# lijun9250lj/video-steganography-PCAMV

Hardware: AMD Instinct MI355X
Metric: 1080p macroblocks/s (embed on) (higher is better)
Workload: dtype u8

## Files before the change

### video-steganography-pcamv_amd/csrc/pcamv_common.h

```cpp
#ifndef PCAMV_COMMON_H
#define PCAMV_COMMON_H
#include <stddef.h>
#include <stdint.h>
#include "../../include/pcamv_gpu.h"
#include "pcamv_variant.h"

#ifdef PCAMV_HOST_EMU
#define PCAMV_DEV static inline
#define PCAMV_CONST static const
#else
#include <hip/hip_runtime.h>
#define PCAMV_DEV __device__ __forceinline__
#define PCAMV_CONST __device__ static const
#endif

#define PCAMV_PAD 32
#define PCAMV_CPAD 16
#define PCAMV_LSW 28
#define PCAMV_LROW 32
#define PCAMV_LSTRIPS(stride) (((stride) + PCAMV_LSW - 1) / PCAMV_LSW + 1)
#define PCAMV_LSTRIP_OF(x) (((uint32_t)(x) * 18725u) >> 19)
#define PCAMV_COST_MAX (1 << 28)
#define PCAMV_COST_MV_LEN (4 * 4 * 2048 + 1)
#define PCAMV_COST_MV_CENTRE (2 * 4 * 2048)
// ... 101 lines not shown
    int nnz_mask;
    uint32_t cxy[64];
    int ccost[192];
    int slots[16];
    uint8_t recb[24 * 16];
    uint8_t recb0[24 * 16];
    uint8_t pred[24 * 16];
    union {
        struct {
            int16_t coef[24][16];
            int16_t cdc[2][4];
            int blk_nz[24], blk_score[24];
            int red[64];
        };
        uint8_t pred4[4][24 * 16];
    };
    int mvc16[9][2];
    int nbc[12];
    uint32_t win[(4 * 480 + 2 * 192) / 4];
    int win_x0, win_y0, win_cx0, win_cy0;
    uint8_t ib_top[3][28];
    uint8_t ib_left[3][16];
    uint8_t nzc[48];
    int16_t cmvd[48][2];
    int8_t i4mode[48];
    int cbp_left, cbp_top;
    int b_fast_intra, fenc_satd_sum, fenc_sa8d_sum;
    uint8_t snap_pred[24 * 16];
    uint8_t snap_nzc[48];
    int16_t snap_cmvd[48][2];
    int snap_cbp_luma, snap_cbp_chroma, snap_nnz_mask;
    int snap_part, snap_cost;
    uint32_t snap_mv[16];
    int snap_ssd, snap_f8r;
#if defined(PCAMV_PROF)
    uint32_t prof_mv[4][16];
    int prof_ntrial;
#endif
#ifdef PCAMV_SEARCH_CALL
    const struct FrameDev *fdesc;
    int me_tmp[10];
    int mvc_tmp[9][2];
#endif
};
#define PCAMV_PASS2_LDS ((int)offsetof(MBLocal, coef))
#define PCAMV_WAVE_LDS_MAX 10240
static_assert(offsetof(MBLocal, pred) + sizeof(((MBLocal *)0)->pred) == offsetof(MBLocal, coef), "pred must end at the second pass' LDS cut");
static_assert(offsetof(MBLocal, fenc) < PCAMV_PASS2_LDS && offsetof(MBLocal, cmv) < PCAMV_PASS2_LDS && offsetof(MBLocal, cref) < PCAMV_PASS2_LDS &&
              offsetof(MBLocal, nnz_mask) < PCAMV_PASS2_LDS && offsetof(MBLocal, slots) + sizeof(((MBLocal *)0)->slots) <= PCAMV_PASS2_LDS &&
              offsetof(MBLocal, ccost) + sizeof(((MBLocal *)0)->ccost) <= PCAMV_PASS2_LDS, "a field the second pass uses lies beyond its LDS");
static_assert(offsetof(MBLocal, ccost) == offsetof(MBLocal, cxy) + sizeof(((MBLocal *)0)->cxy), "cxy and ccost must be contiguous (cab_residual_walk)");
static_assert(offsetof(MBLocal, recb0) == offsetof(MBLocal, recb) + 384 && offsetof(MBLocal, pred) == offsetof(MBLocal, recb) + 768 &&
              offsetof(MBLocal, coef) == offsetof(MBLocal, recb) + 1152, "recb, recb0, pred, the union must be contiguous in this order (TESA_SLOT, L_IFD)");
#define PCAMV_CHAIN_NZ 464
#define PCAMV_CHAIN_MVD 488
#define PCAMV_CHAIN_BYTES 576
#define L_CAB(L, k) ((uint8_t *)(L)->win + 464 * (k))
#define PCAMV_CAB_USED 276
#define L_CABT(L) ((uint8_t *)(L)->win + 464)
#define L_CABK(L) ((uint8_t *)(L)->win + 464 + PCAMV_CAB_USED)
#define L_CTAB(L) ((L)->win + 256)
#define L_IFD(L) ((uint8_t *)(L)->recb)
#define IFD(L, x, y) (L_IFD(L)[((y) + 1) * 32 + (x) + 4])
PCAMV_DEV int scan8_all_of(int idx)
{
    if (idx < 16) return scan8_of(idx);
    if (idx < 24) return 1 + ((idx - 16) & 1) + 8 * (1 + (((idx - 16) >> 1) & 1) + 3 * ((idx - 16) >> 2));
    return 4 + (idx - 24) + 5 * 8;
}

#define TESA_MAX_RANGE 16
#define TESA_REGION_A ((int)((3 * 24 * 16 + 4 * 24 * 16) / 4))
#define TESA_SLOT(L, i) ((i) < TESA_REGION_A ? (uint32_t *)((uint8_t *)(L) + offsetof(MBLocal, recb)) + (i) : (L)->win + ((i) - TESA_REGION_A))
#define TESA_PACK(sad, ry, rx) ((uint32_t)(sad) << 12 | (uint32_t)(ry) << 6 | (uint32_t)(rx))
#define TESA_SAD(e) ((int)((e) >> 12))
#define NB_LEFT 1
#define NB_TOP 2
#define NB_TOPRIGHT 4
#define NB_TOPLEFT 8

#define CAND_PACK(X, Y) ((uint32_t)(uint16_t)(X) | ((uint32_t)(uint16_t)(Y) << 16))
#define CAND_NONE 0x80008000u
#define CAND_X(c) ((int)(int16_t)(L->cxy[c] & 0xffffu))
#define CAND_Y(c) ((int)(int16_t)(L->cxy[c] >> 16))
#define EV_SATD 1
#define EV_CHROMA 2
#define EV_FPEL 4
#define EV_NOMV 8
#define EV_PROBE 16
#define EV_WIN 32
#define EV_SRC4 64
#define WIN_LW 24
#define WIN_LH 20
#define WIN_LP (WIN_LW * WIN_LH)
#define WIN_CW 16
#define WIN_CH 12
#define WIN_CP (WIN_CW * WIN_CH)
struct EvalRes { int cost, idx; };
#ifdef PCAMV_HOST_EMU
#define FOR_CAND(c, n) for (int c = 0; c < (n); c++)
#define NB_SLOT(i) (i)
#else
#define FOR_CAND(c, n) for (int c = LANE(), c##_1 = 1; c##_1 && c < (n); c##_1 = 0)
#define NB_SLOT(i) 0
#endif

#ifdef PCAMV_HOST_EMU
#define NB_ST32(p, v) (*(uint32_t *)(p) = (uint32_t)(v))
#define NB_ST16(p, v) (*(uint16_t *)(p) = (uint16_t)(v))
#define NB_ST8(p, v) (*(int8_t *)(p) = (int8_t)(v))
#define NB_LD32(p) (*(const uint32_t *)(p))
#define NB_LD8(p) (*(const int8_t *)(p))
#define NB_LD16(p) (*(const uint16_t *)(p))
#else
#define NB_ST32(p, v) __hip_atomic_store((uint32_t *)(p), (uint32_t)(v), __ATOMIC_RELAXED, __HIP_MEMORY_SCOPE_AGENT)
#define NB_ST16(p, v) __hip_atomic_store((uint16_t *)(p), (uint16_t)(v), __ATOMIC_RELAXED, __HIP_MEMORY_SCOPE_AGENT)
#define NB_ST8(p, v) __hip_atomic_store((int8_t *)(p), (int8_t)(v), __ATOMIC_RELAXED, __HIP_MEMORY_SCOPE_AGENT)
#define NB_LD32(p) __hip_atomic_load((uint32_t *)(p), __ATOMIC_RELAXED, __HIP_MEMORY_SCOPE_AGENT)
#define NB_LD8(p) __hip_atomic_load((int8_t *)(p), __ATOMIC_RELAXED, __HIP_MEMORY_SCOPE_AGENT)
#define NB_LD16(p) __hip_atomic_load((uint16_t *)(p), __ATOMIC_RELAXED, __HIP_MEMORY_SCOPE_AGENT)
#endif
#define NB_PACK16(lo, hi) ((uint32_t)(uint16_t)(lo) | (uint32_t)(uint16_t)(hi) << 16)

#ifdef PCAMV_HOST_EMU
#define PCAMV_WAVE_SYNC() do { } while (0)
#else
#define PCAMV_WAVE_SYNC() do { __builtin_amdgcn_fence(__ATOMIC_RELEASE, "wavefront"); __builtin_amdgcn_wave_barrier(); \
                               __builtin_amdgcn_fence(__ATOMIC_ACQUIRE, "wavefront"); } while (0)
#endif

struct MEState {
    int i_pixel, xoff, yoff;
    int mvp[2];
    int cost_mv, cost, cost_rec;
    int mv[2];
};


#if defined(PCAMV_PROF) && !defined(PCAMV_HOST_EMU)
#define PCAMV_PROF_N 48
static __device__ unsigned long long pcamv_prof[PCAMV_PROF_N];
__shared__ unsigned long long pcamv_prof_l[PCAMV_PROF_N];
#define PROF_T() __builtin_readcyclecounter()
#define PROF_ADD(i, t0) do { if ((threadIdx.x & 63) == 0) pcamv_prof_l[i] += (unsigned long long)(PROF_T() - (t0)); } while (0)
// ... 12 lines not shown
```

### video-steganography-pcamv_amd/csrc/pcamv_logic.h

```cpp
#ifndef PCAMV_LOGIC_H
#define PCAMV_LOGIC_H
#include "pcamv_common.h"

PCAMV_DEV void cache_mv_set(MBLocal *L, int x, int y, int w, int h, int mvx, int mvy)
{
    PCAMV_WAVE_SYNC();
    FOR_CAND(i, w * h) {
        int j = i / w, k = i - j * w, idx = SCAN8_0 + x + k + 8 * (y + j);
        L->cmv[idx][0] = (int16_t)mvx; L->cmv[idx][1] = (int16_t)mvy;
    }
    PCAMV_WAVE_SYNC();
}
PCAMV_DEV void cache_ref_set(MBLocal *L, int x, int y, int w, int h, int ref)
{
    PCAMV_WAVE_SYNC();
    FOR_CAND(i, w * h) { int j = i / w, k = i - j * w; L->cref[SCAN8_0 + x + k + 8 * (y + j)] = (int8_t)ref; }
    PCAMV_WAVE_SYNC();
}

PCAMV_DEV void predict_from3(int ref, int refa, int refb, int refc, const int16_t *a, const int16_t *b, const int16_t *c, int mvp[2])
{
    int cnt = (refa == ref) + (refb == ref) + (refc == ref);
    if (cnt > 1) { mvp[0] = median3i(a[0], b[0], c[0]); mvp[1] = median3i(a[1], b[1], c[1]); }
    else if (cnt == 1) {
// ... 901 lines not shown
        mvc[2][0] = a->mvc[i + 3][0]; mvc[2][1] = a->mvc[i + 3][1];
        cache_ref_set(L, 2 * i, 0, 2, 4, 0);
        predict_mv(L, 4 * i, 2, me.mvp);
        me_search<VARIANT>(F, L, &me, mvc, 3);
        a->me8x16[i] = me;
        cache_mv_set(L, 2 * i, 0, 2, 4, me.mv[0], me.mv[1]);
    }
    a->cost8x16 = a->me8x16[0].cost + a->me8x16[1].cost;
}
template <int VARIANT>
PCAMV_DEV void analyse_sub8x8(const FrameDev &F, MBLocal *L, Analysis *a, int i8, int pixel)
{
    L->i_partition = PCAMV_D_8x8;
    int n = pixel == PIX_4x4 ? 4 : 2, cost = 0;
    for (int k = 0; k < n; k++) {
        int idx = 4 * i8 + (pixel == PIX_8x4 ? 2 * k : k);
        MEState *me = pixel == PIX_4x4 ? &a->me4x4[i8][k] : pixel == PIX_8x4 ? &a->me8x4[i8][k] : &a->me4x8[i8][k];
        me_setup(me, pixel, 4 * blk_x_of(idx), 4 * blk_y_of(idx));
        predict_mv(L, idx, pixel == PIX_8x4 ? 2 : 1, me->mvp);
        int mvc[1][2];
        const MEState *cand = pixel == PIX_4x4 ? &a->me8x8[i8] : &a->me4x4[i8][0];
        mvc[0][0] = cand->mv[0]; mvc[0][1] = cand->mv[1];
        me_search<VARIANT>(F, L, me, mvc, k == 0);
        cache_mv_set(L, blk_x_of(idx), blk_y_of(idx), pixel == PIX_8x4 ? 2 : 1, pixel == PIX_4x8 ? 2 : 1, me->mv[0], me->mv[1]);
        cost += me->cost;
    }
    cost += F.lambda * (pixel == PIX_4x4 ? 5 : 3);
    if (F.b_chroma_me) {
        int qx[4], qy[4];
        for (int q = 0; q < 4; q++) {
            const MEState *m4 = pixel == PIX_4x4 ? &a->me4x4[i8][q] : pixel == PIX_8x4 ? &a->me8x4[i8][q >> 1] : &a->me4x8[i8][q & 1];
            qx[q] = m4->mv[0]; qy[q] = m4->mv[1];
        }
        cost += prim_chroma4x4_cost(F, L, i8, qx, qy, F.subme > 1);
    }
    if (pixel == PIX_4x4) a->cost4x4[i8] = cost; else if (pixel == PIX_8x4) a->cost8x4[i8] = cost; else a->cost4x8[i8] = cost;
}

PCAMV_DEV int d_mv_x(int i) { return nib64(0x013443101232ull, i) - 2; }
PCAMV_DEV int d_mv_y(int i) { return nib64(0x100134432321ull, i) - 2; }
PCAMV_DEV int d_nb_x(int i) { return nib64(0x122000121ull, i) - 1; }
PCAMV_DEV int d_nb_y(int i) { return nib64(0x120201210ull, i) - 1; }

PCAMV_DEV int rca_nine(const FrameDev &F, MBLocal *L, MEState *me, const uint8_t *enc, int cx, int cy, int nb_cost, int *last, int win)
{
    const int flags = (F.subme > 1 ? EV_SATD : 0) | ((F.b_chroma_me && me->i_pixel <= PIX_8x8) ? EV_CHROMA : 0) | (win ? EV_WIN : 0);
    FOR_CAND(c, 9) L->cxy[c] = CAND_PACK(cx + d_nb_x(c), cy + d_nb_y(c));
    EvalRes r = eval_cands(F, L, me, enc, 9, flags);
    if (nb_cost) { FOR_CAND(c, 9) L->nbc[c] = L->ccost[c]; PCAMV_WAVE_SYNC(); }
    *last = L->ccost[8];
    return r.cost;
}

PCAMV_DEV int rca_mv_cost(const FrameDev &F, MBLocal *L, Analysis *a, MEState *me, int *m_x, int *m_y, int have_base, int win = 0)
{
    const float beta1 = 1.4, beta2 = 4;
    int bmx = me->mv[0], bmy = me->mv[1];
    int cost = 0, min_cost;
    int b_1_neighbor = 0, b_error_pos = 0;
    if (!have_base) { update_cache(L, a); mb_encode(F, L); prim_copy_pred(L, L->recb0); }
    const unsigned long long t_n = PROF_T();
    min_cost = rca_nine(F, L, me, L->recb0, bmx, bmy, 1, &cost, win);
    PROF_ADD(35, t_n);
    me->cost_rec = L->nbc[8];
    const int want_optimal = !(min_cost < me->cost_rec);
    min_cost = PCAMV_COST_MAX; *m_x = 0; *m_y = 0;
    int ii_best = -1;
    if (win) {
        const int flags = (F.subme > 1 ? EV_SATD : 0) | (F.b_chroma_me ? EV_CHROMA : 0) | EV_WIN | EV_SRC4;
        for (int grp = 0; grp < 3; grp++) {
            PROF_CNT(40, 1);
            const unsigned long long t_g = PROF_T();
            for (int j = 0; j < 4; j++) prim_predict_win16(F, L, j, bmx + d_mv_x(4 * grp + j), bmy + d_mv_y(4 * grp + j));
            prim_mb_transform4(F, L);
            PROF_ADD(36, t_g);
            const unsigned long long t_l = PROF_T();
            FOR_CAND(c, 36) {
                int k = c >> 2, ii = 4 * grp + (c & 3);
                L->cxy[c] = CAND_PACK(bmx + d_mv_x(ii) + d_nb_x(k), bmy + d_mv_y(ii) + d_nb_y(k));
            }
            eval_cands(F, L, me, L->pred4[0], 36, flags);
            PROF_ADD(37, t_l);
            for (int j = 0; j < 4; j++) {
                const int ii = 4 * grp + j;
                int min1 = PCAMV_COST_MAX;
                for (int k = 0; k < 9; k++) min1 = imin(min1, L->ccost[4 * k + j]);
                cost = L->ccost[4 * 8 + j];
                int is_opt = (min1 == cost);
                if (is_opt == want_optimal && cost < min_cost) { min_cost = cost; *m_x = d_mv_x(ii); *m_y = d_mv_y(ii); ii_best = ii; }
            }
            if (grp == 0 && min_cost != PCAMV_COST_MAX) break;
        }
    } else
    for (int ii = 0; ii < 12; ii++) {
        PROF_CNT(41, 1);
        int bx1 = bmx + d_mv_x(ii), by1 = bmy + d_mv_y(ii);
        me->mv[0] = bx1; me->mv[1] = by1;
        update_cache(L, a); mb_encode(F, L, win); prim_copy_pred(L, L->recb);
        int min1 = rca_nine(F, L, me, L->recb, bx1, by1, 0, &cost, win);
        int is_opt = (min1 == cost);
        if (is_opt == want_optimal && cost < min_cost) { min_cost = cost; *m_x = d_mv_x(ii); *m_y = d_mv_y(ii); ii_best = ii; }
        if (ii == 3 && min_cost != PCAMV_COST_MAX) break;
    }
    if (min_cost == PCAMV_COST_MAX) {
        b_error_pos = 1; b_1_neighbor = 1;
        *m_x = 0; *m_y = 0;
        for (int k = 0; k < 4; k++) if (L->nbc[k] < min_cost) { min_cost = L->nbc[k]; *m_x = d_nb_x(k); *m_y = d_nb_y(k); }
    } else b_1_neighbor = ii_best <= 3;
    int cost_opt = min_cost > me->cost_rec ? min_cost - me->cost_rec : 1;
    if (!b_1_neighbor) cost_opt = (int)(beta1 * (float)cost_opt);
    else if (b_error_pos) cost_opt = (int)(beta2 * (float)cost_opt);
    me->mv[0] = bmx; me->mv[1] = bmy;
    update_cache(L, a);
    return cost_opt;
}

PCAMV_DEV int carrier_slots(int i_type, int i_partition, const uint8_t *sub, int used, int slots[16])
{
    int n = 0;
    if (!used) return 0;
    if (i_type == PCAMV_P_8x8) {
        for (int i = 0; i < 4; i++)
            switch (sub[i]) {
            case PCAMV_D_L0_8x8: slots[n++] = i * 4; break;
            case PCAMV_D_L0_4x8: slots[n++] = i * 4; slots[n++] = i * 4 + 1; break;
            case PCAMV_D_L0_8x4: slots[n++] = i * 4; slots[n++] = i * 4 + 2; break;
            default: for (int j = 0; j < 4; j++) slots[n++] = i * 4 + j; break;
            }
    } else if (i_type == PCAMV_P_L0) {
        if (i_partition == PCAMV_D_16x16) slots[n++] = 0;
        else if (i_partition == PCAMV_D_8x16) { slots[n++] = 0; slots[n++] = 4; }
        else if (i_partition == PCAMV_D_16x8) { slots[n++] = 0; slots[n++] = 8; }
    }
    return n;
}

PCAMV_DEV int carrier_of_block(int i_type, int i_partition, const uint8_t *sub, int i)
{
    if (i_type == PCAMV_P_8x8) {
        const int i8 = i >> 2, j = i & 3;
        switch (sub[i8]) {
        case PCAMV_D_L0_8x8: return 4 * i8;
        case PCAMV_D_L0_4x8: return 4 * i8 + (j & 1);
        case PCAMV_D_L0_8x4: return 4 * i8 + (j & 2);
        default: return i;
        }
    }
    if (i_partition == PCAMV_D_8x16) return blk_x_of(i) < 2 ? 0 : 4;
    if (i_partition == PCAMV_D_16x8) return blk_y_of(i) < 2 ? 0 : 8;
    return 0;
}

template <int VARIANT>
PCAMV_DEV int analyse_s16(const FrameDev &F, MBLocal *L, Analysis *a)
{
    int b_skip = 0, b_try_pskip = 0;
    for (int i = 0; i < 4; i++) L->sub_part[i] = PCAMV_D_L0_8x8;
    L->i_partition = PCAMV_D_16x16;
    a->rd16x16 = a->cost8x8 = a->cost16x8 = a->cost8x16 = PCAMV_COST_MAX;
    for (int i = 0; i < 4; i++) a->cost4x4[i] = a->cost8x4[i] = a->cost4x8[i] = PCAMV_COST_MAX;
    a->rd16_early = 0;
    L->snap_part = -1; L->snap_cost = PCAMV_COST_MAX;
#if defined(PCAMV_PROF) && !defined(PCAMV_HOST_EMU)
    L->prof_ntrial = 0;
// ... 140 lines not shown
```

### video-steganography-pcamv_amd/csrc/pcamv_mbkernels.h

```cpp
#ifndef PCAMV_MBKERNELS_H
#define PCAMV_MBKERNELS_H
#include "pcamv_logic.h"

#ifdef PCAMV_HOST_EMU
#define PCAMV_LANE0 1
#define PCAMV_RFL(x) (x)
#else
#define PCAMV_LANE0 (LANE() == 0)
#define PCAMV_RFL(x) rfl(x)
#endif

template <int VARIANT>
PCAMV_DEV void mbk_search_finish(const FrameDev &F, MBLocal *L, Analysis *a, int mb_x, int mb_y)
{
    if (MBRD_ON) {
        const unsigned long long t_c = PROF_T();
        L->b_skip_mc = 0;
        const int kept = L->i_type != PCAMV_P_SKIP && L->snap_part == L->i_partition;
        if (kept) prim_rd_restore(F, L);
        else mb_encode(F, L, 0, 1);
#ifdef PCAMV_HOST_EMU
        prim_store_rec(F, L);
#else
        prim_store_rec(F, L, true);
// ... 65 lines not shown
    for (int k = 0; k < n; k++) {
        int s = slots[k], ip, xo, yo;
        MEState *me = slot_me(L, a, s);
        slot_geometry(L->i_type, L->i_partition, L->sub_part, s, &ip, &xo, &yo);
        me_setup(me, ip, xo, yo);
        me->mv[0] = r->mv[s][0]; me->mv[1] = r->mv[s][1];
        me->mvp[0] = FD(F).mvp_aux[(xy * 16 + s) * 2]; me->mvp[1] = FD(F).mvp_aux[(xy * 16 + s) * 2 + 1];
    }
    return n;
}

PCAMV_DEV void mbk_rca(const FrameDev &F, MBLocal *L, Analysis *a, int xy, int k)
{
    if (!FD(F).rec_mb[xy].used) return;
    int *slots = L->slots;
    const int n = analysis_from_record(F, L, a, xy, slots);
    if (k >= n) return;
    MEState *me = slot_me(L, a, slots[k]);
    int dx = 0, dy = 0;
    const int bx = me->mv[0], by = me->mv[1];
    const int cost = rca_mv_cost(F, L, a, me, &dx, &dy, 0);
    if (PCAMV_LANE0) {
        pcamv_mb_t *r = &FD(F).rec_mb[xy];
        r->mv_stego[slots[k]][0] = (int16_t)(bx + dx); r->mv_stego[slots[k]][1] = (int16_t)(by + dy);
        r->inter_stego_cost[slots[k]] = cost;
    }
}

PCAMV_DEV int mbk_recon(const FrameDev &F, MBLocal *L, Analysis *a, int xy, int fused = 0, int have_rec = 0)
{
    const unsigned long long t_e = PROF_T();
    int n;
    if (fused) {
        L->b_skip_mc = 0;
        n = carrier_slots(L->i_type, L->i_partition, L->sub_part, L->i_type != PCAMV_P_SKIP, L->slots);
        for (int k = 0; k < n; k++) { MEState *me = slot_me(L, a, L->slots[k]); me->cost = me->cost_mv = me->cost_rec = 0; }
        if (have_rec) { PROF_ADD(10, t_e); return n; }
    } else {
        n = analysis_from_record(F, L, a, xy, L->slots);
        update_cache(L, a);
    }
    mb_encode(F, L);
    prim_store_rec(F, L);
    if (PCAMV_LANE0 && FD(F).nnz) FD(F).nnz[xy] = (uint16_t)L->nnz_mask;
    PROF_ADD(10, t_e);
    return n;
}
PCAMV_DEV void mbk_rca_all(const FrameDev &F, MBLocal *L, Analysis *a, int xy, int n)
{
    int *slots = L->slots;
    if (FD(F).rec_mb[xy].used && n > 0) {
        const unsigned long long t_w = PROF_T();
        PROF_CNT(42, n);
        prim_copy_pred(L, L->recb0);
        int win = 0;
        if (L->i_type == PCAMV_P_L0 && L->i_partition == PCAMV_D_16x16) {
            const int bx = a->me16x16.mv[0], by = a->me16x16.mv[1];
            if (bx - 3 >= L->mv_min[0] && bx + 3 <= L->mv_max[0] && by - 3 >= L->mv_min[1] && by + 3 <= L->mv_max[1]) { prim_win_load(F, L, bx, by); win = 1; }
        }
        PROF_ADD(34, t_w);
        for (int k = 0; k < n; k++) {
            MEState *me = slot_me(L, a, slots[k]);
            int dx = 0, dy = 0;
            const int bx = me->mv[0], by = me->mv[1];
            const int cost = rca_mv_cost(F, L, a, me, &dx, &dy, 1, win);
            if (PCAMV_LANE0) {
                pcamv_mb_t *r = &FD(F).rec_mb[xy];
                r->mv_stego[slots[k]][0] = (int16_t)(bx + dx); r->mv_stego[slots[k]][1] = (int16_t)(by + dy);
                r->inter_stego_cost[slots[k]] = cost;
            }
        }
    }
}
PCAMV_DEV void mbk_rca_encode(const FrameDev &F, MBLocal *L, Analysis *a, int xy, int fused = 0, int have_rec = 0)
{
    mbk_rca_all(F, L, a, xy, mbk_recon(F, L, a, xy, fused, have_rec));
}

struct P2Pre { const pcamv_mb_t *r; int base, any_flip, nnz1, drain; };
PCAMV_DEV int mbk_pass2(const FrameDev &F, MBLocal *L, int mb_x, int mb_y, int store_rec = 1, const P2Pre *unit = nullptr)
{
    const int xy = mb_y * F.mb_w + mb_x;
    const pcamv_mb_t *r = unit ? unit->r : (const pcamv_mb_t *)L->ccost;
    PCAMV_WAVE_SYNC();
#ifndef PCAMV_HOST_EMU
    uint32_t pre_y = 0, pre_c = 0;
    int any_flip = 1;
    if (unit) any_flip = unit->any_flip;
    else {
        const int lane = LANE();
        if (FD(F).rec_is_pass1) {
            pre_y = *(const uint32_t *)(FD(F).rec[0] + (size_t)(mb_y * 16 + (lane >> 2)) * FD(F).w + mb_x * 16 + (lane & 3) * 4);
            if (lane < 32) pre_c = *(const uint32_t *)(((lane >> 4) ? FD(F).rec[2] : FD(F).rec[1]) + (size_t)(mb_y * 8 + ((lane & 15) >> 1)) * (FD(F).w >> 1) + mb_x * 8 + (lane & 1) * 4);
        }
        if (FD(F).mbflip) any_flip = FD(F).mbflip[xy];
    }
#else
    const int any_flip = 1;
#endif
    if (!unit) {
        FOR_CAND(i, (int)(sizeof(pcamv_mb_t) / 4) + 1) {
            if (i < (int)(sizeof(pcamv_mb_t) / 4)) ((uint32_t *)L->ccost)[i] = ((const uint32_t *)&FD(F).rec_mb[xy])[i];
            else L->ccost[191] = FD(F).car_base ? FD(F).car_base[xy] : 0;
        }
    }
    PCAMV_WAVE_SYNC();
#ifndef PCAMV_HOST_EMU
    if (unit && unit->drain && r->i_type == PCAMV_P_SKIP) asm volatile("s_waitcnt vmcnt(0)" ::: "memory");
#endif
    const int defer_fenc = unit != nullptr && r->i_type != PCAMV_P_SKIP;
    mb_load(F, L, mb_x, mb_y, r->i_type != PCAMV_P_SKIP ? (defer_fenc ? 2 : 1) : 0);
    L->i_type = r->i_type; L->i_partition = r->i_partition;
// ... 73 lines not shown
```

### video-steganography-pcamv_amd/csrc/pcamv_prims_gpu.h

```cpp
#ifndef PCAMV_PRIMS_GPU_H
#define PCAMV_PRIMS_GPU_H
#include "pcamv_common.h"

__device__ __forceinline__ int pcamv_lane_id(void) { int l = (int)(threadIdx.x & 63); asm volatile("" : "+v"(l)); return l; }
#ifndef PCAMV_RD_LO
#define PCAMV_RD_LO 0
#endif
#define LANE() (PCAMV_RD_LO ? (int)(threadIdx.x & 63) : pcamv_lane_id())
__device__ __forceinline__ uint32_t clamp_u8(int v)
{
    asm volatile("" : "+v"(v));
    return (uint32_t)(v < 0 ? 0 : v > 255 ? 255 : v);
}
__device__ __forceinline__ uint32_t ld4u(const uint8_t *p) { uint32_t v; __builtin_memcpy(&v, p, 4); return v; }
__device__ __forceinline__ uint32_t lds4(const uint8_t *p) { return *(const uint32_t *)p; }
__device__ __forceinline__ void sts4(uint8_t *p, uint32_t v) { *(uint32_t *)p = v; }
__device__ __forceinline__ uint32_t avg4(uint32_t a, uint32_t b) { return __builtin_amdgcn_lerp(a, b, 0x01010101u); }
__device__ __forceinline__ int dpp_qp1(int v) { return __builtin_amdgcn_update_dpp(0, v, 0xB1, 0xf, 0xf, false); }
__device__ __forceinline__ int dpp_qp2(int v) { return __builtin_amdgcn_update_dpp(0, v, 0x4E, 0xf, 0xf, false); }
__device__ __forceinline__ int dpp_hmir(int v) { return __builtin_amdgcn_update_dpp(0, v, 0x141, 0xf, 0xf, false); }
__device__ __forceinline__ int dpp_mir(int v) { return __builtin_amdgcn_update_dpp(0, v, 0x140, 0xf, 0xf, false); }

__device__ __forceinline__ int group_sum(int v, int g)
{
// ... 140 lines not shown
    chroma_rows_load(cb, cstride, off, row);
    chroma_block4_rows(row, mvx, mvy, r);
}

__device__ __forceinline__ uint32_t wld4(const MBLocal *L, int b)
{
    const uint32_t *w = L->win + (b >> 2);
    return __builtin_amdgcn_alignbit(w[1], w[0], (uint32_t)(b & 3) * 8u);
}
__device__ __forceinline__ void prim_win_load(const FrameDev &F, MBLocal *L, int bmx, int bmy)
{
    PCAMV_WAVE_SYNC();
    const int lane = LANE();
    const int x0 = L->mb_x * 16 + PCAMV_PAD + ((bmx - 3) >> 2), y0 = L->mb_y * 16 + PCAMV_PAD + ((bmy - 3) >> 2);
    const int cx0 = L->mb_x * 8 + PCAMV_CPAD + ((bmx - 3) >> 3), cy0 = L->mb_y * 8 + PCAMV_CPAD + ((bmy - 3) >> 3);
    const gp8 lb = (gp8)F.luma_base, cb = (gp8)F.chroma_base[0];
    const uint32_t lskip = (uint32_t)F.lskip, psz = (uint32_t)F.plane_size, cstride = (uint32_t)F.cstride, cps = (uint32_t)F.cplane_size;
    for (int i = lane; i < 4 * WIN_LH * (WIN_LW / 4); i += 64) {
        const int pl = i / (WIN_LH * (WIN_LW / 4)), r = (i / (WIN_LW / 4)) % WIN_LH, c = i % (WIN_LW / 4);
        L->win[i] = gld4(lb, (uint32_t)pl * psz + (uint32_t)(y0 + r) * PCAMV_LROW + lsw_x((uint32_t)(x0 + 4 * c), lskip));
    }
    for (int i = lane; i < 2 * WIN_CH * (WIN_CW / 4); i += 64) {
        const int pl = i / (WIN_CH * (WIN_CW / 4)), r = (i / (WIN_CW / 4)) % WIN_CH, c = i % (WIN_CW / 4);
        L->win[4 * WIN_LP / 4 + i] = gld4(cb, (uint32_t)pl * cps + (uint32_t)(cy0 + r) * cstride + (uint32_t)(cx0 + 4 * c));
    }
    if (lane == 0) { L->win_x0 = x0; L->win_y0 = y0; L->win_cx0 = cx0; L->win_cy0 = cy0; }
    PCAMV_WAVE_SYNC();
}
__device__ __forceinline__ void chroma_block4_win(const MBLocal *L, int b, int mvx, int mvy, uint32_t r[4])
{
    const int dx = mvx & 7, dy = mvy & 7;
    const uint32_t W = mul24u(8 - dx, 8 - dy) | mul24u(dx, 8 - dy) << 8 | mul24u(8 - dx, dy) << 16 | mul24u(dx, dy) << 24;
    const uint32_t sh = (uint32_t)(b & 3) * 8u;
    uint32_t w[5][4];
#pragma unroll
    for (int k = 0; k < 5; k++) {
        const uint32_t *p = L->win + ((b + k * WIN_CW) >> 2);
        const uint32_t lo = __builtin_amdgcn_alignbit(p[1], p[0], sh), hi = __builtin_amdgcn_alignbit(p[2], p[1], sh);
        w[k][0] = lo; w[k][1] = __builtin_amdgcn_alignbit(hi, lo, 8); w[k][2] = __builtin_amdgcn_alignbit(hi, lo, 16); w[k][3] = __builtin_amdgcn_alignbit(hi, lo, 24);
    }
#pragma unroll
    for (int k = 0; k < 4; k++) {
        uint32_t o = 0;
#pragma unroll
        for (int i = 0; i < 4; i++) {
            const uint32_t px = __builtin_amdgcn_perm(w[k + 1][i], w[k][i], 0x05040100u);
            o |= (__builtin_amdgcn_udot4(px, W, 32u, false) >> 6) << (8 * i);
        }
        r[k] = o;
    }
}

struct EvalEnv { const int16_t *cost_mv; const uint8_t *luma_base, *chroma_base; long long plane_size, cplane_size; int lskip, cstride; int *trace; int trace_mb; };
__device__ __forceinline__ EvalRes eval_list_body(const EvalEnv &F, MBLocal *L, const uint8_t *enc, int ip_, int xoff_, int yoff_,
                                                  int n_, int flags_, int mvp0_, int mvp1_)
{
    const int ip = rfl(ip_), xoff = rfl(xoff_), yoff = rfl(yoff_), n = rfl(n_), flags = rfl(flags_), mvp0 = rfl(mvp0_), mvp1 = rfl(mvp1_);
    const int lane = LANE();
    const int lgn = lg_nblk_of(ip), lgw = lg_w4_of(ip), nblk = 1 << lgn;
    const int satd = flags & EV_SATD;
    const gp8 cost_tab = (gp8)(F.cost_mv - PCAMV_COST_MV_CENTRE);
    PCAMV_WAVE_SYNC();
    const unsigned long long t_ev = PROF_T();
    PROF_CNT(32, 1); PROF_CNT(33, n);
    int key_acc = 0x7fffffff;
    {
        const int slot = lane >> lgn, blk = lane & (nblk - 1);
        const int px = xoff + 4 * (blk & ((1 << lgw) - 1)), py = yoff + 4 * (blk >> lgw);
        uint32_t e[4], ec[8];
        const uint8_t *encl = (flags & EV_SRC4) ? enc + (slot & 3) * 384 : enc;
#pragma unroll
        for (int k = 0; k < 4; k++) e[k] = lds4(encl + (py + k) * 16 + px);
        if (satd) pk_cols(e, ec);
        const gp8 lb = (gp8)F.luma_base;
        const uint32_t stride = PCAMV_LROW, psz = (uint32_t)F.plane_size, lskip = (uint32_t)F.lskip;
        const gp8 lb1 = lb + stride, lb2 = lb1 + stride, lb3 = lb2 + stride;
        const uint32_t rowbase = (uint32_t)(L->mb_y * 16 + py + PCAMV_PAD) * stride, colbase = (uint32_t)(L->mb_x * 16 + px + PCAMV_PAD);
        const int cpp = 64 >> lgn;
        for (int p0 = 0; p0 < n; p0 += cpp) {
            const int c = p0 + slot;
            const uint32_t xy = L->cxy[c < n ? c : 0];
            const bool act = c < n && xy != CAND_NONE;
            const int mvx = act ? (int)(int16_t)(xy & 0xffffu) : 0, mvy = act ? (int)(int16_t)(xy >> 16) : 0;
            const uint32_t o = rowbase + (uint32_t)((mvy >> 2) * (int)stride) + lsw_x(colbase + (uint32_t)(mvx >> 2), lskip);
            int mvb0 = 0, mvb1 = 0;
            if (!(flags & EV_NOMV)) { mvb0 = gld_cost(cost_tab, (uint32_t)(mvx - mvp0 + PCAMV_COST_MV_CENTRE)); mvb1 = gld_cost(cost_tab, (uint32_t)(mvy - mvp1 + PCAMV_COST_MV_CENTRE)); }
            uint32_t r[4];
            if (flags & EV_WIN) {
                const int dx = mvx & 3, dy = mvy & 3;
                const int wb = (L->mb_y * 16 + py + PCAMV_PAD + (mvy >> 2) - L->win_y0) * WIN_LW + (L->mb_x * 16 + px + PCAMV_PAD + (mvx >> 2) - L->win_x0);
                const int ba = wb + ((dx != 0) + 2 * (dy == 2)) * WIN_LP + (dy == 3 ? WIN_LW : 0);
#pragma unroll
                for (int k = 0; k < 4; k++) r[k] = wld4(L, ba + k * WIN_LW);
                if ((dx | dy) & 1) {
                    const int bb = wb + (dy ? (2 + (dx == 2)) * WIN_LP : 0) + (dx == 3);
#pragma unroll
                    for (int k = 0; k < 4; k++) r[k] = avg4(r[k], wld4(L, bb + k * WIN_LW));
                }
            } else if (flags & EV_FPEL) {
                r[0] = gld4(lb, o); r[1] = gld4(lb1, o); r[2] = gld4(lb2, o); r[3] = gld4(lb3, o);
            } else {
                const int dx = mvx & 3, dy = mvy & 3;
                const uint32_t oa = o + (dx != 0 ? psz : 0u) + (dy == 2 ? 2u * psz : 0u) + (dy == 3 ? stride : 0u);
                r[0] = gld4(lb, oa); r[1] = gld4(lb1, oa); r[2] = gld4(lb2, oa); r[3] = gld4(lb3, oa);
                if ((dx | dy) & 1) {
                    const uint32_t ob = o + (dy ? (dx == 2 ? 3u * psz : 2u * psz) : 0u) + (dx == 3);
                    r[0] = avg4(r[0], gld4(lb, ob)); r[1] = avg4(r[1], gld4(lb1, ob));
                    r[2] = avg4(r[2], gld4(lb2, ob)); r[3] = avg4(r[3], gld4(lb3, ob));
                }
            }
            asm volatile("" : "+v"(mvb0), "+v"(mvb1), "+v"(r[0]), "+v"(r[1]), "+v"(r[2]), "+v"(r[3]));
            int v;
            if (satd) v = satd4x4_half(ec, r);
            else {
                uint32_t sa = 0;
#pragma unroll
                for (int k = 0; k < 4; k++) sa = __builtin_amdgcn_sad_u8(e[k], r[k], sa);
                v = (int)sa;
            }
            v = group_sum(v, nblk) + mvb0 + mvb1;
            if (blk == 0 && c < n) L->ccost[c] = act ? v : PCAMV_COST_MAX;
            if (blk == 0 && act) key_acc = imin(key_acc, (v << 6) | c);
        }
    }
    PCAMV_WAVE_SYNC();
    if ((flags & EV_CHROMA) && ip <= PIX_8x8) {
        const int lgnb = lgn - 2, nb = 1 << lgnb, lgcw = lgw - 1;
        const int slot = lane >> (lgnb + 1), plane = (lane >> lgnb) & 1, blk = lane & (nb - 1);
        const int px = (xoff >> 1) + 4 * (blk & ((1 << lgcw) - 1)), py = (yoff >> 1) + 4 * (blk >> lgcw);
        uint32_t e[4], ec[8];
        const uint8_t *encl = (flags & EV_SRC4) ? enc + (slot & 3) * 384 : enc;
#pragma unroll
        for (int k = 0; k < 4; k++) e[k] = lds4(encl + 256 + (py + k) * 16 + plane * 8 + px);
        if (satd) pk_cols(e, ec);
        const gp8 cb = (gp8)F.chroma_base;
        const uint32_t cstride = (uint32_t)F.cstride;
        const uint32_t rowbase = (plane ? (uint32_t)F.cplane_size : 0u) + mul24u((uint32_t)(L->mb_y * 8 + py + PCAMV_CPAD), cstride) + (uint32_t)(L->mb_x * 8 + px + PCAMV_CPAD);
        const int cpp = 64 >> (lgnb + 1);
        for (int p0 = 0; p0 < n; p0 += cpp) {
            const int c = p0 + slot;
            const uint32_t xy = L->cxy[c < n ? c : 0];
            const bool act = c < n && xy != CAND_NONE;
            const int mvx = act ? (int)(int16_t)(xy & 0xffffu) : 0, mvy = act ? (int)(int16_t)(xy >> 16) : 0;
            uint32_t r[4];
            if (flags & EV_WIN)
                chroma_block4_win(L, 4 * WIN_LP + plane * WIN_CP + (L->mb_y * 8 + py + PCAMV_CPAD + (mvy >> 3) - L->win_cy0) * WIN_CW
                                         + (L->mb_x * 8 + px + PCAMV_CPAD + (mvx >> 3) - L->win_cx0), mvx, mvy, r);
            else
                chroma_block4(cb, cstride, rowbase + (uint32_t)(mul24s(mvy >> 3, (int)cstride) + (mvx >> 3)), mvx, mvy, r);
            int v;
            if (satd) v = satd4x4_half(ec, r);
            else {
                uint32_t sa = 0;
#pragma unroll
                for (int k = 0; k < 4; k++) sa = __builtin_amdgcn_sad_u8(e[k], r[k], sa);
                v = (int)sa;
            }
            v = group_sum(v, nb);
            if (blk == 0 && act) {
                if (flags & EV_PROBE) L->ccost[64 * (1 + plane) + c] = v;
                else atomicAdd(&L->ccost[c], v);
            }
        }
    }
    PCAMV_WAVE_SYNC();
    int key = 0x7fffffff;
    if ((flags & EV_CHROMA) && ip <= PIX_8x8) { if (lane < n) { int cc = L->ccost[lane]; if (cc < PCAMV_COST_MAX) key = (cc << 6) | lane; } }
    else key = key_acc;
    key = wave_min_i32(key);
    EvalRes res;
    if (key == 0x7fffffff) { res.cost = PCAMV_COST_MAX; res.idx = -1; }
    else { res.cost = key >> 6; res.idx = key & 63; }
    PROF_ADD(38, t_ev);
#ifdef PCAMV_TRACE
    if (F.trace && L->mb_xy == F.trace_mb && lane == 0)
        for (int c = 0; c < n; c++) {
            if (L->cxy[c] == CAND_NONE) continue;
            int k = F.trace[0];
            if (k < 4000) { int *t = F.trace + 1 + 8 * k; t[0] = ip; t[1] = xoff; t[2] = yoff; t[3] = CAND_X(c); t[4] = CAND_Y(c); t[5] = flags | ((enc == L->recb || enc == L->recb0) ? 32 : 0); t[6] = L->ccost[c]; t[7] = c; F.trace[0] = k + 1; }
        }
#endif
    PCAMV_WAVE_SYNC();
    return res;
}

__device__ __forceinline__ EvalRes prim_eval_list(const FrameDev &F, MBLocal *L, const uint8_t *enc, int ip, int xoff, int yoff, int n, int flags, int mvp0, int mvp1)
{
    EvalEnv E;
    E.cost_mv = F.cost_mv; E.luma_base = F.luma_base; E.chroma_base = F.chroma_base[0]; E.plane_size = F.plane_size; E.cplane_size = F.cplane_size;
    E.lskip = F.lskip; E.cstride = F.cstride; E.trace = F.trace; E.trace_mb = F.trace_mb;
    return eval_list_body(E, L, enc, ip, xoff, yoff, n, flags, mvp0, mvp1);
}

__device__ __forceinline__ EvalRes prim_esa_window(const FrameDev &F, MBLocal *L, int ip_, int xoff_, int yoff_, int min_x_, int min_y_,
                                                   int width_, int nrows_, int mvp0_, int mvp1_)
{
    const int ip = rfl(ip_), xoff = rfl(xoff_), yoff = rfl(yoff_), min_x = rfl(min_x_), min_y = rfl(min_y_), width = rfl(width_), nrows = rfl(nrows_);
    const int mvp0 = rfl(mvp0_), mvp1 = rfl(mvp1_);
    const int lane = LANE();
    const int lgn = lg_nblk_of(ip), lgw = lg_w4_of(ip), nblk = 1 << lgn;
    const int slot = lane >> lgn, blk = lane & (nblk - 1), nslot = 64 >> lgn;
    const int px = xoff + 4 * (blk & ((1 << lgw) - 1)), py = yoff + 4 * (blk >> lgw);
    const gp8 cost_tab = (gp8)(F.cost_mv - PCAMV_COST_MV_CENTRE);
    PCAMV_WAVE_SYNC();
    uint32_t e[4];
#pragma unroll
    for (int k = 0; k < 4; k++) e[k] = lds4(L->fenc + (py + k) * 16 + px);
    const gp8 lb = (gp8)F.luma_raster;
    const uint32_t stride = (uint32_t)F.stride;
    const gp8 lb1 = lb + stride, lb2 = lb1 + stride, lb3 = lb2 + stride;
    const uint32_t rowbase = (uint32_t)(L->mb_y * 16 + py + PCAMV_PAD) * stride + (uint32_t)(L->mb_x * 16 + px + PCAMV_PAD);
    int best = 0x7fffffff;
    for (int r0 = 0; r0 < nrows; r0 += nslot) {
        const int ry = r0 + slot;
        const bool rowok = ry < nrows;
        const int my = min_y + (rowok ? ry : 0);
        const int ycost = gld_cost(cost_tab, (uint32_t)(my * 4 - mvp1 + PCAMV_COST_MV_CENTRE));
        const uint32_t orow = rowbase + (uint32_t)(my * (int)stride + min_x);
        for (int x0 = 0; x0 < width; x0 += 4) {
            const uint32_t o = orow + (uint32_t)x0;
            const uint64_t w0 = gld8(lb, o), w1 = gld8(lb1, o), w2 = gld8(lb2, o), w3 = gld8(lb3, o);
            uint32_t s[4];
#pragma unroll
            for (int j = 0; j < 4; j++) {
                const uint32_t sh = 8u * (uint32_t)j;
                uint32_t a = 0;
                a = __builtin_amdgcn_sad_u8(e[0], j ? __builtin_amdgcn_alignbit((uint32_t)(w0 >> 32), (uint32_t)w0, sh) : (uint32_t)w0, a);
                a = __builtin_amdgcn_sad_u8(e[1], j ? __builtin_amdgcn_alignbit((uint32_t)(w1 >> 32), (uint32_t)w1, sh) : (uint32_t)w1, a);
                a = __builtin_amdgcn_sad_u8(e[2], j ? __builtin_amdgcn_alignbit((uint32_t)(w2 >> 32), (uint32_t)w2, sh) : (uint32_t)w2, a);
                a = __builtin_amdgcn_sad_u8(e[3], j ? __builtin_amdgcn_alignbit((uint32_t)(w3 >> 32), (uint32_t)w3, sh) : (uint32_t)w3, a);
                s[j] = a;
            }
            int p01 = (int)(s[0] | s[1] << 16), p23 = (int)(s[2] | s[3] << 16);
            p01 = group_sum(p01, nblk); p23 = group_sum(p23, nblk);
            const int jn = nblk >= 4 ? 1 : 4;
            for (int jj = 0; jj < jn; jj++) {
                const int j = nblk >= 4 ? (blk & 3) : jj;
                const int sad = (j & 2 ? p23 : p01) >> (16 * (j & 1)) & 0xffff;
                const int mx = min_x + x0 + j;
                const int cost = sad + ycost + gld_cost(cost_tab, (uint32_t)(mx * 4 - mvp0 + PCAMV_COST_MV_CENTRE));
                const int key = (cost << 11) | (ry * width + x0 + j);
                if (rowok && x0 + j < width && key < best) best = key;
            }
        }
// ... 529 lines not shown
    (void)F;
    PCAMV_WAVE_SYNC();
}
__device__ __forceinline__ void prim_mb_transform4(const FrameDev &F, MBLocal *L)
{
    const auto &Q = FD(F);
    PCAMV_WAVE_SYNC();
    const int lane = LANE();
    {
        const int j = lane >> 4, blk = lane & 15, px = 4 * blk_x_of(blk), py = 4 * blk_y_of(blk);
        uint8_t *pr = L->pred4[j];
        int16_t d[16]; int nz, score, rawdc;
        residual_block_at(F, L, pr, px, py, true, d, &nz, &score, &rawdc);
        const int sc = (nz && Q.b_dct_decimate) ? score : 0;
        int q8 = sc + dpp_qp1(sc); q8 += dpp_qp2(q8);
        int any8 = nz | dpp_qp1(nz); any8 |= dpp_qp2(any8);
        int row = q8 + dpp_hmir(q8); row += dpp_mir(row);
        const bool keep = Q.b_dct_decimate ? (q8 >= 4 && row >= 6) : any8 != 0;
        if (keep && nz) idct4x4_add(pr + py * 16 + px, d);
    }
    if (lane < 32) {
        const int j = lane >> 3, ch = (lane >> 2) & 1, ci = lane & 3, px = ch * 8 + (ci & 1) * 4, py = 16 + (ci >> 1) * 4;
        uint8_t *pr = L->pred4[j];
        int16_t d[16]; int nz, score, rawdc;
        residual_block_at(F, L, pr, px, py, false, d, &nz, &score, &rawdc);
        const int sc = (nz && Q.b_dct_decimate) ? score : 0;
        int q8 = sc + dpp_qp1(sc); q8 += dpp_qp2(q8);
        int any8 = nz | dpp_qp1(nz); any8 |= dpp_qp2(any8);
        const int cdc = quad_had2x2(rawdc, ci);
        int dcq;
        { const int mf = Q.q_mf[1][0] >> 1, bias = Q.q_bias[1][0] << 1;
          dcq = cdc > 0 ? ((bias + cdc) * mf >> 16) : -((bias - cdc) * mf >> 16); }
        int nzdc = dcq != 0; nzdc |= dpp_qp1(nzdc); nzdc |= dpp_qp2(nzdc);
        int dmf = Q.dq_mf_c[0], qbits = Q.chroma_qp / 6 - 5;
        if (qbits > 0) { dmf <<= qbits; qbits = 0; }
        const int rdc = (int16_t)(quad_had2x2(dcq, ci) * dmf >> -qbits);
        const int cmode = (q8 < 7 && Q.b_dct_decimate) || !any8 ? (nzdc ? 1 : 0) : 2;
        uint8_t *dst = pr + py * 16 + px;
        if (cmode == 2) { if (nzdc) d[0] = (int16_t)rdc; idct4x4_add(dst, d); }
        else if (cmode == 1) {
            const int v = (rdc + 32) >> 6;
#pragma unroll
            for (int y = 0; y < 4; y++) {
                uint32_t p = lds4(dst + y * 16), o = 0;
#pragma unroll
                for (int x = 0; x < 4; x++) o |= (uint32_t)clip3i((int)((p >> (8 * x)) & 255) + v, 0, 255) << (8 * x);
                sts4(dst + y * 16, o);
            }
        }
    }
    PCAMV_WAVE_SYNC();
}

__device__ __forceinline__ int prim_chroma_ssd(const FrameDev &F, MBLocal *L, int ch)
{
    PCAMV_WAVE_SYNC();
    const int lane = LANE();
    int v = 0;
    if (lane < 16) {
        int row = lane >> 1, c4 = lane & 1;
        uint32_t e = lds4(L->fenc + 256 + row * 16 + ch * 8 + c4 * 4), p = lds4(L->pred + 256 + row * 16 + ch * 8 + c4 * 4);
#pragma unroll
        for (int x = 0; x < 4; x++) { int dd = (int)((e >> (8 * x)) & 255) - (int)((p >> (8 * x)) & 255); v += dd * dd; }
    }
    v = group_sum(v, 16);
    (void)F;
    return __builtin_amdgcn_readlane(v, 0);
}
__device__ __forceinline__ void prim_copy_pred(MBLocal *L, uint8_t *dst)
{
    PCAMV_WAVE_SYNC();
    const int lane = LANE();
    ((uint32_t *)dst)[lane] = ((const uint32_t *)L->pred)[lane];
    if (lane < 32) ((uint32_t *)dst)[64 + lane] = ((const uint32_t *)L->pred)[64 + lane];
    PCAMV_WAVE_SYNC();
}
__device__ __forceinline__ void prim_store_rec(const FrameDev &F, MBLocal *L, bool wt = false)
{
    const auto &D = FD(F);
    PCAMV_WAVE_SYNC();
    const int lane = LANE();
    { int row = lane >> 2, c4 = lane & 3;
      uint32_t *d = (uint32_t *)(D.rec[0] + (size_t)(L->mb_y * 16 + row) * D.w + L->mb_x * 16 + c4 * 4);
      const uint32_t v = lds4(L->pred + row * 16 + c4 * 4);
      if (wt) NB_ST32(d, v); else *d = v; }
    if (lane < 32) {
        int plane = lane >> 4, row = (lane & 15) >> 1, c4 = lane & 1;
        uint32_t *d = (uint32_t *)((plane ? D.rec[2] : D.rec[1]) + (size_t)(L->mb_y * 8 + row) * (D.w >> 1) + L->mb_x * 8 + c4 * 4);
        const uint32_t v = lds4(L->pred + 256 + row * 16 + plane * 8 + c4 * 4);
        if (wt) NB_ST32(d, v); else *d = v;
    }
}
__device__ __forceinline__ void prim_load_rec(const FrameDev &F, MBLocal *L)
{
    const auto &D = FD(F);
    PCAMV_WAVE_SYNC();
    const int lane = LANE();
    { int row = lane >> 2, c4 = lane & 3;
      sts4(L->pred + row * 16 + c4 * 4, *(const uint32_t *)(D.rec[0] + (size_t)(L->mb_y * 16 + row) * D.w + L->mb_x * 16 + c4 * 4)); }
    if (lane < 32) {
        int plane = lane >> 4, row = (lane & 15) >> 1, c4 = lane & 1;
        sts4(L->pred + 256 + row * 16 + plane * 8 + c4 * 4, *(const uint32_t *)((plane ? D.rec[2] : D.rec[1]) + (size_t)(L->mb_y * 8 + row) * (D.w >> 1) + L->mb_x * 8 + c4 * 4));
    }
    PCAMV_WAVE_SYNC();
}
__device__ __forceinline__ void prim_store_mvr(const FrameDev &F, MBLocal *L, int mvx, int mvy)
// ... 7 lines not shown
```

### video-steganography-pcamv_amd/csrc/pcamv_tesa.hip

```cpp
#include <hip/hip_runtime.h>
#include <stdint.h>
#include "pcamv_flow.hip.h"

static __global__ void __launch_bounds__(64, PCAMV_FLOW_OCC) k_analyse_flow_tesa(const FrameDev *__restrict__ Fs, FlowDev fl)
{
    __shared__ MBLocal L;
    __shared__ Analysis A;
    flow_loop<0, V_TESA>(Fs, fl, L, &A, nullptr);
}

void pcamv_launch_flow_tesa(unsigned waves, hipStream_t st, const FrameDev *dF, const FlowDev &fl)
{
    hipLaunchKernelGGL(k_analyse_flow_tesa, dim3(waves), dim3(64), 0, st, dF, fl);
}
```

Measured before the change: 25.59 million.

## Fuse RCA nine-neighbour head into first window group and fold minima across lanes

When the search window is loaded, the separate nine-neighbour evaluation is appended to the first group's 36-candidate evaluation. The source block switches mid-list to the reconstructed prediction placed right in front of pred4. The per-group minimum scans over LDS are replaced by a DPP/swizzle cross-lane reduction, and the pred-to-recb0 copy plus the trailing cache update are skipped on the window path. This removes one eval pass, a copy and serial LDS loops, at the cost of layout assumptions and variant-specific macros; the TESA variant opts out of all three.

```diff
diff --git a/video-steganography-pcamv_amd/csrc/pcamv_common.h b/video-steganography-pcamv_amd/csrc/pcamv_common.h
--- a/video-steganography-pcamv_amd/csrc/pcamv_common.h
+++ b/video-steganography-pcamv_amd/csrc/pcamv_common.h
@@ -177,6 +177,7 @@
 static_assert(offsetof(MBLocal, ccost) == offsetof(MBLocal, cxy) + sizeof(((MBLocal *)0)->cxy), "cxy and ccost must be contiguous (cab_residual_walk)");
 static_assert(offsetof(MBLocal, recb0) == offsetof(MBLocal, recb) + 384 && offsetof(MBLocal, pred) == offsetof(MBLocal, recb) + 768 &&
               offsetof(MBLocal, coef) == offsetof(MBLocal, recb) + 1152, "recb, recb0, pred, the union must be contiguous in this order (TESA_SLOT, L_IFD)");
+static_assert(offsetof(MBLocal, pred4) == offsetof(MBLocal, pred) + 384, "pred must lie right in front of pred4[0] (EV_SRC5)");
 #define PCAMV_CHAIN_NZ 464
 #define PCAMV_CHAIN_MVD 488
 #define PCAMV_CHAIN_BYTES 576
@@ -215,6 +216,8 @@
 #define EV_PROBE 16
 #define EV_WIN 32
 #define EV_SRC4 64
+#define EV_SRC5 128
+#define RCA_HEAD 36
 #define WIN_LW 24
 #define WIN_LH 20
 #define WIN_LP (WIN_LW * WIN_LH)
diff --git a/video-steganography-pcamv_amd/csrc/pcamv_logic.h b/video-steganography-pcamv_amd/csrc/pcamv_logic.h
--- a/video-steganography-pcamv_amd/csrc/pcamv_logic.h
+++ b/video-steganography-pcamv_amd/csrc/pcamv_logic.h
@@ -977,6 +977,22 @@
     return r.cost;
 }
 
+#if !defined(PCAMV_HOST_EMU) && !defined(PCAMV_RCA_NO_FUSED_HEAD)
+#define RCA_FUSED_HEAD 1
+#else
+#define RCA_FUSED_HEAD 0
+#endif
+#if !defined(PCAMV_HOST_EMU) && !defined(PCAMV_RCA_NO_LANE_FOLD)
+#define RCA_LANE_FOLD 1
+#else
+#define RCA_LANE_FOLD 0
+#endif
+#ifdef PCAMV_RCA_KEEP_COPY
+#define RCA_BASE(L, win) ((L)->recb0)
+#else
+#define RCA_BASE(L, win) ((win) ? (L)->pred : (L)->recb0)
+#endif
+
 PCAMV_DEV int rca_mv_cost(const FrameDev &F, MBLocal *L, Analysis *a, MEState *me, int *m_x, int *m_y, int have_base, int win = 0)
 {
     const float beta1 = 1.4, beta2 = 4;
@@ -984,33 +1000,61 @@
     int cost = 0, min_cost;
     int b_1_neighbor = 0, b_error_pos = 0;
     if (!have_base) { update_cache(L, a); mb_encode(F, L); prim_copy_pred(L, L->recb0); }
-    const unsigned long long t_n = PROF_T();
-    min_cost = rca_nine(F, L, me, L->recb0, bmx, bmy, 1, &cost, win);
-    PROF_ADD(35, t_n);
-    me->cost_rec = L->nbc[8];
-    const int want_optimal = !(min_cost < me->cost_rec);
+    const int fused = RCA_FUSED_HEAD && win;
+    int want_optimal = 0;
+    if (!fused) {
+        const unsigned long long t_n = PROF_T();
+        min_cost = rca_nine(F, L, me, RCA_BASE(L, win), bmx, bmy, 1, &cost, win);
+        PROF_ADD(35, t_n);
+        me->cost_rec = L->nbc[8];
+        want_optimal = !(min_cost < me->cost_rec);
+    }
     min_cost = PCAMV_COST_MAX; *m_x = 0; *m_y = 0;
     int ii_best = -1;
     if (win) {
         const int flags = (F.subme > 1 ? EV_SATD : 0) | (F.b_chroma_me ? EV_CHROMA : 0) | EV_WIN | EV_SRC4;
         for (int grp = 0; grp < 3; grp++) {
+            const int head = fused && grp == 0;
             PROF_CNT(40, 1);
             const unsigned long long t_g = PROF_T();
             for (int j = 0; j < 4; j++) prim_predict_win16(F, L, j, bmx + d_mv_x(4 * grp + j), bmy + d_mv_y(4 * grp + j));
             prim_mb_transform4(F, L);
             PROF_ADD(36, t_g);
             const unsigned long long t_l = PROF_T();
-            FOR_CAND(c, 36) {
-                int k = c >> 2, ii = 4 * grp + (c & 3);
-                L->cxy[c] = CAND_PACK(bmx + d_mv_x(ii) + d_nb_x(k), bmy + d_mv_y(ii) + d_nb_y(k));
+            const int n = head ? RCA_HEAD + 9 : RCA_HEAD;
+            FOR_CAND(c, n) {
+                const int hd = c >= RCA_HEAD, k = hd ? c - RCA_HEAD : c >> 2, ii = 4 * grp + (c & 3);
+                L->cxy[c] = CAND_PACK(bmx + (hd ? 0 : d_mv_x(ii)) + d_nb_x(k), bmy + (hd ? 0 : d_mv_y(ii)) + d_nb_y(k));
             }
-            eval_cands(F, L, me, L->pred4[0], 36, flags);
+#if RCA_FUSED_HEAD
+            prim_eval_list<true>(F, L, L->pred4[0], me->i_pixel, me->xoff, me->yoff, n, head ? flags | EV_SRC5 : flags, me->mvp[0], me->mvp[1]);
+#else
+            eval_cands(F, L, me, L->pred4[0], n, flags);
+#endif
             PROF_ADD(37, t_l);
+#if RCA_LANE_FOLD
+            const RcaFold f = prim_rca_fold(L, head);
+            if (head) { me->cost_rec = f.cost_rec; want_optimal = !f.nb_less; }
+#else
+            if (head) {
+                FOR_CAND(c, 9) L->nbc[c] = L->ccost[RCA_HEAD + c];
+                PCAMV_WAVE_SYNC();
+                me->cost_rec = L->nbc[8];
+                int minh = PCAMV_COST_MAX;
+                for (int k = 0; k < 9; k++) minh = imin(minh, L->nbc[k]);
+                want_optimal = !(minh < me->cost_rec);
+            }
+#endif
             for (int j = 0; j < 4; j++) {
                 const int ii = 4 * grp + j;
+#if RCA_LANE_FOLD
+                const int min1 = f.min1[j];
+                cost = f.cost[j];
+#else
                 int min1 = PCAMV_COST_MAX;
                 for (int k = 0; k < 9; k++) min1 = imin(min1, L->ccost[4 * k + j]);
                 cost = L->ccost[4 * 8 + j];
+#endif
                 int is_opt = (min1 == cost);
                 if (is_opt == want_optimal && cost < min_cost) { min_cost = cost; *m_x = d_mv_x(ii); *m_y = d_mv_y(ii); ii_best = ii; }
             }
@@ -1035,6 +1079,9 @@
     int cost_opt = min_cost > me->cost_rec ? min_cost - me->cost_rec : 1;
     if (!b_1_neighbor) cost_opt = (int)(beta1 * (float)cost_opt);
     else if (b_error_pos) cost_opt = (int)(beta2 * (float)cost_opt);
+#ifndef PCAMV_RCA_KEEP_COPY
+    if (win) return cost_opt;
+#endif
     me->mv[0] = bmx; me->mv[1] = bmy;
     update_cache(L, a);
     return cost_opt;
diff --git a/video-steganography-pcamv_amd/csrc/pcamv_mbkernels.h b/video-steganography-pcamv_amd/csrc/pcamv_mbkernels.h
--- a/video-steganography-pcamv_amd/csrc/pcamv_mbkernels.h
+++ b/video-steganography-pcamv_amd/csrc/pcamv_mbkernels.h
@@ -141,12 +141,15 @@
     if (FD(F).rec_mb[xy].used && n > 0) {
         const unsigned long long t_w = PROF_T();
         PROF_CNT(42, n);
-        prim_copy_pred(L, L->recb0);
         int win = 0;
         if (L->i_type == PCAMV_P_L0 && L->i_partition == PCAMV_D_16x16) {
             const int bx = a->me16x16.mv[0], by = a->me16x16.mv[1];
             if (bx - 3 >= L->mv_min[0] && bx + 3 <= L->mv_max[0] && by - 3 >= L->mv_min[1] && by + 3 <= L->mv_max[1]) { prim_win_load(F, L, bx, by); win = 1; }
         }
+#ifndef PCAMV_RCA_KEEP_COPY
+        if (!win)
+#endif
+        prim_copy_pred(L, L->recb0);
         PROF_ADD(34, t_w);
         for (int k = 0; k < n; k++) {
             MEState *me = slot_me(L, a, slots[k]);
diff --git a/video-steganography-pcamv_amd/csrc/pcamv_prims_gpu.h b/video-steganography-pcamv_amd/csrc/pcamv_prims_gpu.h
--- a/video-steganography-pcamv_amd/csrc/pcamv_prims_gpu.h
+++ b/video-steganography-pcamv_amd/csrc/pcamv_prims_gpu.h
@@ -216,6 +216,7 @@
 }
 
 struct EvalEnv { const int16_t *cost_mv; const uint8_t *luma_base, *chroma_base; long long plane_size, cplane_size; int lskip, cstride; int *trace; int trace_mb; };
+template <bool SRC5 = false>
 __device__ __forceinline__ EvalRes eval_list_body(const EvalEnv &F, MBLocal *L, const uint8_t *enc, int ip_, int xoff_, int yoff_,
                                                   int n_, int flags_, int mvp0_, int mvp1_)
 {
@@ -243,6 +244,11 @@
         const int cpp = 64 >> lgn;
         for (int p0 = 0; p0 < n; p0 += cpp) {
             const int c = p0 + slot;
+            if (SRC5 && (flags & EV_SRC5) && c >= RCA_HEAD && c - cpp < RCA_HEAD) {
+#pragma unroll
+                for (int k = 0; k < 4; k++) e[k] = lds4(enc - 384 + (py + k) * 16 + px);
+                if (satd) pk_cols(e, ec);
+            }
             const uint32_t xy = L->cxy[c < n ? c : 0];
             const bool act = c < n && xy != CAND_NONE;
             const int mvx = act ? (int)(int16_t)(xy & 0xffffu) : 0, mvy = act ? (int)(int16_t)(xy >> 16) : 0;
@@ -303,6 +309,11 @@
         const int cpp = 64 >> (lgnb + 1);
         for (int p0 = 0; p0 < n; p0 += cpp) {
             const int c = p0 + slot;
+            if (SRC5 && (flags & EV_SRC5) && c >= RCA_HEAD && c - cpp < RCA_HEAD) {
+#pragma unroll
+                for (int k = 0; k < 4; k++) e[k] = lds4(enc - 384 + 256 + (py + k) * 16 + plane * 8 + px);
+                if (satd) pk_cols(e, ec);
+            }
             const uint32_t xy = L->cxy[c < n ? c : 0];
             const bool act = c < n && xy != CAND_NONE;
             const int mvx = act ? (int)(int16_t)(xy & 0xffffu) : 0, mvy = act ? (int)(int16_t)(xy >> 16) : 0;
@@ -348,12 +359,13 @@
     return res;
 }
 
+template <bool SRC5 = false>
 __device__ __forceinline__ EvalRes prim_eval_list(const FrameDev &F, MBLocal *L, const uint8_t *enc, int ip, int xoff, int yoff, int n, int flags, int mvp0, int mvp1)
 {
     EvalEnv E;
     E.cost_mv = F.cost_mv; E.luma_base = F.luma_base; E.chroma_base = F.chroma_base[0]; E.plane_size = F.plane_size; E.cplane_size = F.cplane_size;
     E.lskip = F.lskip; E.cstride = F.cstride; E.trace = F.trace; E.trace_mb = F.trace_mb;
-    return eval_list_body(E, L, enc, ip, xoff, yoff, n, flags, mvp0, mvp1);
+    return eval_list_body<SRC5>(E, L, enc, ip, xoff, yoff, n, flags, mvp0, mvp1);
 }
 
 __device__ __forceinline__ EvalRes prim_esa_window(const FrameDev &F, MBLocal *L, int ip_, int xoff_, int yoff_, int min_x_, int min_y_,
@@ -989,6 +1001,31 @@
     PCAMV_WAVE_SYNC();
 }
 
+struct RcaFold { int min1[4], cost[4], cost_rec, nb_less; };
+__device__ __forceinline__ RcaFold prim_rca_fold(MBLocal *L, int head)
+{
+    const int lane = LANE();
+    const int v = lane < RCA_HEAD + 9 ? L->ccost[lane] : PCAMV_COST_MAX;
+    int m = lane < RCA_HEAD ? v : PCAMV_COST_MAX;
+    m = imin(m, __builtin_amdgcn_update_dpp(0, m, 0x124, 0xf, 0xf, false));
+    m = imin(m, __builtin_amdgcn_update_dpp(0, m, 0x128, 0xf, 0xf, false));
+    m = imin(m, __builtin_amdgcn_ds_swizzle(m, 0x401f));
+    RcaFold f;
+#pragma unroll
+    for (int j = 0; j < 4; j++) {
+        f.cost[j] = __builtin_amdgcn_readlane(m, 32 + j);
+        f.min1[j] = imin(__builtin_amdgcn_readlane(m, j), f.cost[j]);
+    }
+    f.cost_rec = 0; f.nb_less = 0;
+    if (head) {
+        f.cost_rec = __builtin_amdgcn_readlane(v, RCA_HEAD + 8);
+        f.nb_less = __ballot(lane >= RCA_HEAD && lane < RCA_HEAD + 8 && v < f.cost_rec) != 0;
+        if (lane >= RCA_HEAD && lane < RCA_HEAD + 9) L->nbc[lane - RCA_HEAD] = v;
+        PCAMV_WAVE_SYNC();
+    }
+    return f;
+}
+
 __device__ __forceinline__ int prim_chroma_ssd(const FrameDev &F, MBLocal *L, int ch)
 {
     PCAMV_WAVE_SYNC();
diff --git a/video-steganography-pcamv_amd/csrc/pcamv_tesa.hip b/video-steganography-pcamv_amd/csrc/pcamv_tesa.hip
--- a/video-steganography-pcamv_amd/csrc/pcamv_tesa.hip
+++ b/video-steganography-pcamv_amd/csrc/pcamv_tesa.hip
@@ -1,5 +1,8 @@
 #include <hip/hip_runtime.h>
 #include <stdint.h>
+#define PCAMV_RCA_NO_FUSED_HEAD 1
+#define PCAMV_RCA_NO_LANE_FOLD 1
+#define PCAMV_RCA_KEEP_COPY 1
 #include "pcamv_flow.hip.h"
 
 static __global__ void __launch_bounds__(64, PCAMV_FLOW_OCC) k_analyse_flow_tesa(const FrameDev *__restrict__ Fs, FlowDev fl)
```

New measurement: 25.81 million, median of 6. No clear change (+0.9%).
